# syl051088/DynaAlign

Measured on AMD Instinct MI355X. Metric: sequence-pairs/sec (MinHash k=4 n_hash=500; NW BLOSUM62) at 1/2/4/8 MI355X, higher is better.
Workload: dtype u32

## Files before the change

### dynaalign_amd/csrc/dict_kernels.hip

```cpp
#include "da_common.hpp"
#include <atomic>

namespace da {
namespace {

__global__ __launch_bounds__(256) void k_sig_transpose(const uint32_t *__restrict__ sig, int64_t ld_sig, int64_t n,
                                                       int n_hash, uint32_t *__restrict__ sigT, int64_t ldT) {
  __shared__ uint32_t t[64][65];
  const int64_t i0 = (int64_t)blockIdx.x * 64;
  const int h0 = blockIdx.y * 64;
  const int lx = threadIdx.x & 63, ly = threadIdx.x >> 6;
  for (int r = ly; r < 64; r += 4) {
    const int64_t i = i0 + r;
    const int h = h0 + lx;
    t[r][lx] = (i < n && h < n_hash) ? sig[i * ld_sig + h] : 0u;
  }
  __syncthreads();
  for (int r = ly; r < 64; r += 4) {
    const int h = h0 + r;
    const int64_t i = i0 + lx;
    if (h < n_hash && i < ldT) sigT[(int64_t)h * ldT + i] = t[lx][r];
  }
}

constexpr int DK_THREADS = 1024;
constexpr int DK_SLOTS = 16384;
constexpr int DK_PART_KEYS = 8192;
constexpr int DK_MAX_PARTS = 16;

__device__ __forceinline__ uint32_t dk_mix(uint32_t x) {
  x ^= x >> 16; x *= 0x85ebca6bu; x ^= x >> 13; x *= 0xc2b2ae35u; x ^= x >> 16;
  return x;
}
__device__ __forceinline__ int dk_part(uint32_t z, int R) { return (int)__umulhi(z, (uint32_t)R); }
__device__ __forceinline__ uint32_t dk_slot(uint32_t z) { return (z * 0x9e3779b1u) >> (32 - 14); }
static_assert(DK_SLOTS == (1 << 14), "dk_slot assumes 2^14 slots");

__global__ __launch_bounds__(DK_THREADS) void k_dictionary(const uint32_t *__restrict__ sigT, int64_t ldT, int64_t n,
                                                           int R, uint32_t *__restrict__ szT, uint32_t *__restrict__ siT,
                                                           uint16_t *__restrict__ idsT, int64_t ld_ids,
                                                           int *__restrict__ status) {
  constexpr int NW = DK_THREADS / 64;
  __shared__ uint32_t keys[DK_SLOTS];
  __shared__ uint16_t vals[DK_SLOTS];
  __shared__ uint32_t wsum[NW];
  __shared__ uint32_t cnt[NW][DK_MAX_PARTS];
  __shared__ uint32_t pbase[DK_MAX_PARTS + 1];
  const int tid = threadIdx.x, lane = tid & 63, wave = tid >> 6;
  const uint32_t *col = sigT + (int64_t)blockIdx.x * ldT;
  uint32_t *sz = szT + (int64_t)blockIdx.x * ldT;
  uint32_t *si = siT + (int64_t)blockIdx.x * ldT;
  uint16_t *ids = idsT + (int64_t)blockIdx.x * ld_ids;

  for (int t = tid; t < NW * DK_MAX_PARTS; t += DK_THREADS) (&cnt[0][0])[t] = 0;
  __syncthreads();
  for (int64_t i = tid; i < n; i += DK_THREADS) atomicAdd(&cnt[wave][dk_part(dk_mix(col[i]), R)], 1u);
  __syncthreads();
  if (tid < R) {
    uint32_t run = 0;
    for (int w = 0; w < NW; ++w) { const uint32_t c = cnt[w][tid]; cnt[w][tid] = run; run += c; }
    pbase[tid + 1] = run;
  }
  __syncthreads();
  if (tid == 0) {
    pbase[0] = 0;
    for (int p = 0; p < R; ++p) pbase[p + 1] += pbase[p];
  }
  __syncthreads();
  for (int64_t i = tid; i < n; i += DK_THREADS) {
    const uint32_t z = dk_mix(col[i]);
    const int p = dk_part(z, R);
    const uint32_t pos = pbase[p] + atomicAdd(&cnt[wave][p], 1u);
    sz[pos] = z;
    si[pos] = (uint32_t)i;
  }
  __syncthreads();

  uint32_t base = 0;
  bool overflow = false;
  for (int r = 0; r < R; ++r) {
    const uint32_t lo = pbase[r], hi = pbase[r + 1];
    const uint32_t q = (uint32_t)((r + 1) % R);
    const uint32_t EMPTY = (uint32_t)((((uint64_t)q << 32) + (uint32_t)R - 1) / (uint32_t)R);
    for (int s = tid; s < DK_SLOTS; s += DK_THREADS) { keys[s] = EMPTY; vals[s] = 0; }
    __syncthreads();
    for (uint32_t j = lo + tid; j < hi; j += DK_THREADS) {
      const uint32_t z = sz[j];
      uint32_t s = dk_slot(z);
      for (int probes = 0;; ++probes) {
        const uint32_t old = atomicCAS(&keys[s], EMPTY, z);
        if (old == EMPTY) break;
        if (old == z) { vals[s] = 1; break; }
        s = (s + 1) & (DK_SLOTS - 1);
        if (probes >= DK_SLOTS) { overflow = true; break; }
      }
    }
    __syncthreads();

    uint32_t mine = 0;
    for (int s = tid; s < DK_SLOTS; s += DK_THREADS) mine += vals[s];
    uint32_t incl = mine;
    for (int o = 1; o < 64; o <<= 1) {
      const uint32_t up = __shfl_up(incl, o);
      if (lane >= o) incl += up;
    }
    if (lane == 63) wsum[wave] = incl;
    __syncthreads();
    uint32_t before = 0, total = 0;
    for (int w = 0; w < NW; ++w) {
      const uint32_t v = wsum[w];
      if (w < wave) before += v;
      total += v;
    }
    uint32_t next = base + before + incl - mine;
    for (int s = tid; s < DK_SLOTS; s += DK_THREADS) {
      if (keys[s] == EMPTY) continue;
      vals[s] = vals[s] ? (uint16_t)(next++) : (uint16_t)0xFFFFu;
    }
    base += total;
    __syncthreads();

    for (uint32_t j = lo + tid; j < hi; j += DK_THREADS) {
      const uint32_t z = sz[j];
      uint32_t s = dk_slot(z);
      uint16_t id = 0xFFFFu;
      for (int probes = 0; probes <= DK_SLOTS; ++probes) {
        const uint32_t cur = keys[s];
        if (cur == z) { id = vals[s]; break; }
        if (cur == EMPTY) break;
        s = (s + 1) & (DK_SLOTS - 1);
      }
      ids[si[j]] = id;
    }
    __syncthreads();
  }
  if (overflow) atomicMax(status, 1);
  if (tid == 0 && base > 65534u) atomicMax(status, 2);
  if (tid == 0) atomicMax(status + 1, (int)base);
}

__global__ __launch_bounds__(1024) void k_hy_split(const uint16_t *__restrict__ idsT, int64_t ld_ids, int n, int max_ids, int keep,
                                                   uint16_t *__restrict__ idsD, uint16_t *__restrict__ idsS, unsigned long long *__restrict__ stats) {
  extern __shared__ uint32_t hy_hist[];
  uint32_t *part = hy_hist + max_ids;
  __shared__ uint32_t red[16];
  const int tid = threadIdx.x, lane = tid & 63, wave = tid >> 6;
  const uint16_t *ids = idsT + (int64_t)blockIdx.x * ld_ids;
  uint16_t *outD = idsD + (int64_t)blockIdx.x * ld_ids, *outS = idsS + (int64_t)blockIdx.x * ld_ids;
  for (int c = tid; c < max_ids; c += 1024) hy_hist[c] = 0;
  __syncthreads();
  const uint4 *ids8 = reinterpret_cast<const uint4 *>(ids);
  const int n8 = (n + 7) / 8;
  for (int q = tid; q < n8; q += 1024) {
    const uint4 v = ids8[q];
    const uint32_t w[4] = {v.x, v.y, v.z, v.w};
#pragma unroll
    for (int u = 0; u < 8; ++u) {
      const uint32_t c = (w[u >> 1] >> (16 * (u & 1))) & 0xffffu;
      if (q * 8 + u < n && c != 0xFFFFu) atomicAdd(&hy_hist[c], 1u);
    }
  }
  __syncthreads();
  auto count_ge = [&](uint32_t t) -> uint32_t {
    uint32_t k = 0;
    for (int c = tid; c < max_ids; c += 1024) k += hy_hist[c] >= t;
    for (int o = 32; o > 0; o >>= 1) k += __shfl_down(k, o);
    __syncthreads();
    if (lane == 0) red[wave] = k;
    __syncthreads();
    uint32_t tot = 0;
    for (int w = 0; w < 16; ++w) tot += red[w];
    return tot;
  };
  uint32_t lo = 1, hi = (uint32_t)n + 1u;
  while (lo < hi) {
    const uint32_t mid = lo + (hi - lo) / 2;
    if (count_ge(mid) <= (uint32_t)keep) hi = mid; else lo = mid + 1;
  }
  const uint32_t t = lo, above = count_ge(t), quota = (uint32_t)keep - above;
  const bool ties = t >= 3;
  const int per = (max_ids + 1023) / 1024, c_lo = tid * per, c_hi = c_lo + per < max_ids ? c_lo + per : max_ids;
  uint32_t f1 = 0, f2 = 0;
  for (int c = c_lo; c < c_hi; ++c) { const uint32_t m = hy_hist[c]; f1 += m >= t; f2 += ties && m == t - 1; }
  part[tid] = (f1 << 16) | f2;
  __syncthreads();
  if (tid < 64) {
    uint32_t v[16], tot = 0;
#pragma unroll
    for (int q = 0; q < 16; ++q) { v[q] = part[tid * 16 + q]; tot += v[q]; }
    uint32_t incl = tot;
    for (int o = 1; o < 64; o <<= 1) { const uint32_t up = __shfl_up(incl, o); if (tid >= o) incl += up; }
    uint32_t run = incl - tot;
#pragma unroll
    for (int q = 0; q < 16; ++q) { part[tid * 16 + q] = run; run += v[q]; }
  }
  __syncthreads();
  uint32_t p1 = part[tid] >> 16, p2 = part[tid] & 0xffffu;
  unsigned long long e = 0, mx = 0, e_all = 0, mx_all = 0;
  for (int c = c_lo; c < c_hi; ++c) {
    const uint32_t m = hy_hist[c];
    uint32_t rank = 0xFFFFu;
    if (m >= t) rank = p1++;
    else if (ties && m == t - 1) { if (p2 < quota) rank = above + p2; ++p2; }
    if (m >= 2) {
      const unsigned long long inc = (unsigned long long)m * (m - 1) / 2;
      e_all += inc; mx_all = m > mx_all ? m : mx_all;
      if (rank == 0xFFFFu) { e += inc; mx = m > mx ? m : mx; }
    }
    hy_hist[c] = rank;
  }
  for (int o = 32; o > 0; o >>= 1) {
    e += __shfl_down(e, o);
    e_all += __shfl_down(e_all, o);
    const unsigned long long other = __shfl_down(mx, o), other_all = __shfl_down(mx_all, o);
    mx = other > mx ? other : mx;
    mx_all = other_all > mx_all ? other_all : mx_all;
  }
  if (lane == 0) { atomicAdd(&stats[0], e); atomicMax(&stats[1], mx); atomicAdd(&stats[2], e_all); atomicMax(&stats[3], mx_all); }
  __syncthreads();
  uint4 *outD8 = reinterpret_cast<uint4 *>(outD), *outS8 = reinterpret_cast<uint4 *>(outS);
  for (int q = tid; q < n8; q += 1024) {
    const uint4 v = ids8[q];
    const uint32_t w[4] = {v.x, v.y, v.z, v.w};
    uint32_t d[4] = {0, 0, 0, 0}, sp[4] = {0, 0, 0, 0};
#pragma unroll
    for (int u = 0; u < 8; ++u) {
      const uint32_t c = (w[u >> 1] >> (16 * (u & 1))) & 0xffffu;
      const bool live = q * 8 + u < n && c != 0xFFFFu;
      const uint32_t r = live ? hy_hist[c] : 0xFFFFu;
      d[u >> 1] |= r << (16 * (u & 1));
      sp[u >> 1] |= ((live && r == 0xFFFFu) ? c : 0xFFFFu) << (16 * (u & 1));
    }
    outD8[q] = make_uint4(d[0], d[1], d[2], d[3]);
    outS8[q] = make_uint4(sp[0], sp[1], sp[2], sp[3]);
  }
}

__global__ __launch_bounds__(256) void k_ids_to_planes(const uint16_t *__restrict__ idsT, int64_t ld_ids, int64_t n,
                                                       int n_hash, int pl, int code_bits, uint32_t *__restrict__ planes) {
  __shared__ uint16_t tile[64][66];
  const int64_t i0 = (int64_t)blockIdx.x * 64;
  const int lane = threadIdx.x & 63, wave = threadIdx.x >> 6;
  const PlaneGeom pg = plane_geom(n, n_hash, pl);
  const int ngroup = (n_hash + 31) / 32;
  for (int h0 = 0; h0 < ngroup * 32; h0 += 64) {
    __syncthreads();
    for (int r = wave; r < 64; r += 4) {
      const int h = h0 + r;
      const int64_t i = i0 + lane;
      tile[r][lane] = (h < n_hash && i < n) ? idsT[(int64_t)h * ld_ids + i] : (uint16_t)0;
    }
    __syncthreads();
    for (int sq = wave; sq < 64; sq += 4) {
      const int64_t i = i0 + sq;
      if (i >= n) break;
      const uint32_t v = tile[lane][sq];
      const bool single = (v == 0xFFFFu) && (h0 + lane < n_hash);
      const uint32_t va = single ? (1u << code_bits) - 2u : v;
      const uint32_t vb = single ? (1u << code_bits) - 1u : v;
      uint32_t wa = 0, wb = 0;
      for (int p = 0; p < pl; ++p) {
        const unsigned long long m = __ballot((va >> p) & 1u);
        const uint32_t half = (lane < 32) ? (uint32_t)m : (uint32_t)(m >> 32);
        wa = ((lane & 31) == p) ? half : wa;
      }
      {
        const unsigned long long m = __ballot(vb & 1u);
        const uint32_t half = (lane < 32) ? (uint32_t)m : (uint32_t)(m >> 32);
        wb = ((lane & 31) == 0) ? half : wa;
      }
      const int g = (h0 >> 5) + (lane >> 5);
      const int p = lane & 31;
      if (p < pl && g < ngroup) {
        const int64_t w = plane_unit_word(pg, i, g, p >> 2);
        planes[w + (p & 3)] = wa;
        planes[pg.copy_words + w + ((p & 3) ^ 1)] = wb;
        if (pl == 16) {
          const int64_t ws = pad16_base_words(n, n_hash) + pad16_slot_word(n, n_hash, i, g);
          planes[ws + p] = wa;
          planes[ws + pad16_copy_words(n, n_hash) + (p ^ 1)] = wb;
        }
      }
    }
  }
}

__global__ __launch_bounds__(256) void k_sig_to_planes(const uint32_t *__restrict__ sig, int64_t ld_sig, int64_t n,
                                                       int n_hash, uint32_t *__restrict__ planes) {
  const int lane = threadIdx.x & 63, wave = threadIdx.x >> 6;
  const int64_t i = (int64_t)blockIdx.x * 4 + wave;
  if (i >= n) return;
  const PlaneGeom pg = plane_geom(n, n_hash, 32);
  const int ngroup = (n_hash + 31) / 32;
  const uint32_t *row = sig + i * ld_sig;
  for (int h0 = 0; h0 < ngroup * 32; h0 += 64) {
    const int h = h0 + lane;
    const uint32_t v = (h < n_hash) ? row[h] : 0u;
    uint32_t w = 0;
#pragma unroll
    for (int p = 0; p < 32; ++p) {
      const unsigned long long m = __ballot((v >> p) & 1u);
      const uint32_t half = (lane < 32) ? (uint32_t)m : (uint32_t)(m >> 32);
      w = ((lane & 31) == p) ? half : w;
    }
    const int g = (h0 >> 5) + (lane >> 5);
    const int p = lane & 31;
    if (g < ngroup) {
      const int64_t u = plane_unit_word(pg, i, 2 * g + (p >> 4), (p & 15) >> 2);
      planes[u + (p & 3)] = w;
      planes[pg.copy_words + u + ((p & 3) ^ 1)] = w;
    }
  }
}

}

static int64_t dict_ldT(int64_t n) { return ceil_div(n, 64) * 64; }

struct DictWork { uint32_t *sigT, *sz, *si; uint16_t *idsT; int *status; };
static DictWork dict_work(void *d_work, int64_t n, int n_hash) {
  const size_t m = (size_t)n_hash * (size_t)dict_ldT(n);
  DictWork w;
  w.sigT = static_cast<uint32_t *>(d_work);
  w.sz = w.sigT + m;
  w.si = w.sz + m;
  w.idsT = reinterpret_cast<uint16_t *>(w.si + m);
  w.status = reinterpret_cast<int *>((reinterpret_cast<uintptr_t>(w.idsT + m) + 63) & ~(uintptr_t)63);
  return w;
}

size_t mh_planes_workspace_bytes(int64_t n, int n_hash) {
  if (n <= 0 || n_hash <= 0 || n > DA_DICT_MAX_N) return 256;
  const size_t ldT = (size_t)dict_ldT(n);
  return (size_t)n_hash * ldT * (4 + 4 + 4 + 2) + 256;
}

const uint16_t *mh_dictionary_codes(const void *d_work, int64_t n, int n_hash, int64_t *ld_ids) {
  *ld_ids = dict_ldT(n);
  return dict_work(const_cast<void *>(d_work), n, n_hash).idsT;
}

int launch_mh_dictionary(const uint32_t *d_sig, int64_t ld_sig, int64_t n, int n_hash, void *d_work,
                         int **d_status_out, hipStream_t stream) {
  const int64_t ldT = dict_ldT(n);
  const DictWork w = dict_work(d_work, n, n_hash);
  uint32_t *sigT = w.sigT;
  uint16_t *idsT = w.idsT;
  int *status = w.status;
  *d_status_out = status;
  DA_HIP_TRY(hipMemsetAsync(status, 0, 2 * sizeof(int), stream));
  hipLaunchKernelGGL(k_sig_transpose, dim3((unsigned)ceil_div(n, 64), (unsigned)ceil_div(n_hash, 64)), dim3(256), 0,
                     stream, d_sig, ld_sig, n, n_hash, sigT, ldT);
  int R = (int)ceil_div(n, DK_PART_KEYS);
  if (R < 2) R = 2;
  hipLaunchKernelGGL(k_dictionary, dim3((unsigned)n_hash), dim3(DK_THREADS), 0, stream, sigT, ldT, n, R, w.sz, w.si, idsT, ldT,
                     status);
  DA_HIP_TRY(hipGetLastError());
  return DA_OK;
}

constexpr int HY_MAX_IDS = 32768;
int launch_mh_heavy_split(void *d_work, int64_t n, int n_hash, int max_ids, int keep, const uint16_t **d_dense_out, const uint16_t **d_sparse_out,
                          unsigned long long *d_stats, hipStream_t stream) {
  if (max_ids < 1 || max_ids > HY_MAX_IDS || keep < 1 || keep > 65534 || n > 0x7fffffffLL)
    return fail(DA_ERR_UNSUPPORTED, "heavy / rare split: too many repeated values per column");
  const int64_t ldT = dict_ldT(n);
  const DictWork w = dict_work(d_work, n, n_hash);
  uint16_t *dense = reinterpret_cast<uint16_t *>(w.sz), *sparse = reinterpret_cast<uint16_t *>(w.si);
  static std::atomic<uint64_t> attr_done;
  int dev = 0;
  DA_HIP_TRY(hipGetDevice(&dev));
  if (!((attr_done.load() >> (dev & 63)) & 1u)) {
    DA_HIP_TRY(hipFuncSetAttribute(reinterpret_cast<const void *>(k_hy_split), hipFuncAttributeMaxDynamicSharedMemorySize, (HY_MAX_IDS + 1024) * 4));
    attr_done.fetch_or(1ull << (dev & 63));
  }
  DA_HIP_TRY(hipMemsetAsync(d_stats, 0, 32, stream));
  hipLaunchKernelGGL(k_hy_split, dim3((unsigned)n_hash), dim3(1024), (size_t)(max_ids + 1024) * 4, stream, w.idsT, ldT, (int)n, max_ids, keep, dense, sparse,
                     d_stats);
  DA_HIP_TRY(hipGetLastError());
  *d_dense_out = dense;
  *d_sparse_out = sparse;
  return DA_OK;
}

int mh_plane_bits_for(int max_ids) {
  if (max_ids + 2 <= (1 << 8)) return 8;
  if (max_ids + 2 <= (1 << 12)) return 12;
  if (max_ids + 2 <= (1 << 14)) return 14;
  if (max_ids + 2 <= (1 << 15)) return 15;
  return 16;
}

int launch_ids_to_planes(const void *d_work, int64_t n, int n_hash, int plane_bits, uint32_t *d_planes,
                         hipStream_t stream, const uint16_t *d_codes) {
  const int64_t ldT = dict_ldT(n);
  const uint16_t *idsT = d_codes ? d_codes : dict_work(const_cast<void *>(d_work), n, n_hash).idsT;
  hipLaunchKernelGGL(k_ids_to_planes, dim3((unsigned)ceil_div(n, 64)), dim3(256), 0, stream, idsT, ldT, n, n_hash,
                     (plane_bits == 14 || plane_bits == 15) ? 16 : plane_bits, plane_bits, d_planes);
  DA_HIP_TRY(hipGetLastError());
  return DA_OK;
}

int launch_sig_to_planes(const uint32_t *d_sig, int64_t ld_sig, int64_t n, int n_hash, uint32_t *d_planes,
                         hipStream_t stream) {
  hipLaunchKernelGGL(k_sig_to_planes, dim3((unsigned)ceil_div(n, 4)), dim3(256), 0, stream, d_sig, ld_sig, n, n_hash,
                     d_planes);
  DA_HIP_TRY(hipGetLastError());
  return DA_OK;
}

}
```

Before: 355.3 billion.

## Vectorize and batch global loads in dictionary build and ids-to-planes transpose

Replaces the scalar strided global reads in the dictionary kernel's histogram, scatter, insert and emit phases with batched uint4 loads. Several loads are issued before processing so more memory requests are in flight, and unaligned head and tail elements get separate handling. The ids-to-planes kernel now loads 16-byte units and prefetches the next 64-row tile into registers while the current one is processed. DK_MAX_PARTS is now derived from DA_DICT_MAX_N. Risks include misaligned vector loads if the leading dimensions are not multiples of four, reading past n into padding in the planes kernel, and higher register pressure.

```diff
diff --git a/dynaalign_amd/csrc/dict_kernels.hip b/dynaalign_amd/csrc/dict_kernels.hip
--- a/dynaalign_amd/csrc/dict_kernels.hip
+++ b/dynaalign_amd/csrc/dict_kernels.hip
@@ -24,17 +24,19 @@
 }
 
 constexpr int DK_THREADS = 1024;
-constexpr int DK_SLOTS = 16384;
-constexpr int DK_PART_KEYS = 8192;
-constexpr int DK_MAX_PARTS = 16;
+constexpr int DK_SLOT_BITS = 14;
+constexpr int DK_SLOTS = 1 << DK_SLOT_BITS;
+constexpr int DK_PART_KEYS = DK_SLOTS / 2;
+constexpr int DK_MAX_PARTS = (DA_DICT_MAX_N + DK_PART_KEYS - 1) / DK_PART_KEYS;
+constexpr int DK_COL_BATCH = 8;
+constexpr int DK_PART_BATCH = 4;
 
 __device__ __forceinline__ uint32_t dk_mix(uint32_t x) {
   x ^= x >> 16; x *= 0x85ebca6bu; x ^= x >> 13; x *= 0xc2b2ae35u; x ^= x >> 16;
   return x;
 }
 __device__ __forceinline__ int dk_part(uint32_t z, int R) { return (int)__umulhi(z, (uint32_t)R); }
-__device__ __forceinline__ uint32_t dk_slot(uint32_t z) { return (z * 0x9e3779b1u) >> (32 - 14); }
-static_assert(DK_SLOTS == (1 << 14), "dk_slot assumes 2^14 slots");
+__device__ __forceinline__ uint32_t dk_slot(uint32_t z) { return (z * 0x9e3779b1u) >> (32 - DK_SLOT_BITS); }
 
 __global__ __launch_bounds__(DK_THREADS) void k_dictionary(const uint32_t *__restrict__ sigT, int64_t ldT, int64_t n,
                                                            int R, uint32_t *__restrict__ szT, uint32_t *__restrict__ siT,
@@ -54,7 +56,25 @@
 
   for (int t = tid; t < NW * DK_MAX_PARTS; t += DK_THREADS) (&cnt[0][0])[t] = 0;
   __syncthreads();
-  for (int64_t i = tid; i < n; i += DK_THREADS) atomicAdd(&cnt[wave][dk_part(dk_mix(col[i]), R)], 1u);
+  const uint4 *col4 = reinterpret_cast<const uint4 *>(col);
+  const int nv = (int)(n >> 2);
+  const int n_tail = (int)n - 4 * nv;
+  for (int q0 = 0; q0 < nv; q0 += DK_THREADS * DK_COL_BATCH) {
+    uint4 v[DK_COL_BATCH];
+#pragma unroll
+    for (int b = 0; b < DK_COL_BATCH; ++b) {
+      const int q = q0 + b * DK_THREADS + tid;
+      v[b] = col4[q < nv ? q : 0];
+    }
+#pragma unroll
+    for (int b = 0; b < DK_COL_BATCH; ++b) {
+      if (q0 + b * DK_THREADS + tid >= nv) continue;
+      const uint32_t x[4] = {v[b].x, v[b].y, v[b].z, v[b].w};
+#pragma unroll
+      for (int c = 0; c < 4; ++c) atomicAdd(&cnt[wave][dk_part(dk_mix(x[c]), R)], 1u);
+    }
+  }
+  if (tid < n_tail) atomicAdd(&cnt[wave][dk_part(dk_mix(col[4 * nv + tid]), R)], 1u);
   __syncthreads();
   if (tid < R) {
     uint32_t run = 0;
@@ -67,13 +87,30 @@
     for (int p = 0; p < R; ++p) pbase[p + 1] += pbase[p];
   }
   __syncthreads();
-  for (int64_t i = tid; i < n; i += DK_THREADS) {
-    const uint32_t z = dk_mix(col[i]);
+  auto scatter = [&](uint32_t x, uint32_t i) {
+    const uint32_t z = dk_mix(x);
     const int p = dk_part(z, R);
     const uint32_t pos = pbase[p] + atomicAdd(&cnt[wave][p], 1u);
     sz[pos] = z;
-    si[pos] = (uint32_t)i;
-  }
+    si[pos] = i;
+  };
+  for (int q0 = 0; q0 < nv; q0 += DK_THREADS * DK_COL_BATCH) {
+    uint4 v[DK_COL_BATCH];
+#pragma unroll
+    for (int b = 0; b < DK_COL_BATCH; ++b) {
+      const int q = q0 + b * DK_THREADS + tid;
+      v[b] = col4[q < nv ? q : 0];
+    }
+#pragma unroll
+    for (int b = 0; b < DK_COL_BATCH; ++b) {
+      const int q = q0 + b * DK_THREADS + tid;
+      if (q >= nv) continue;
+      const uint32_t x[4] = {v[b].x, v[b].y, v[b].z, v[b].w};
+#pragma unroll
+      for (int c = 0; c < 4; ++c) scatter(x[c], (uint32_t)(4 * q + c));
+    }
+  }
+  if (tid < n_tail) scatter(col[4 * nv + tid], (uint32_t)(4 * nv + tid));
   __syncthreads();
 
   uint32_t base = 0;
@@ -84,9 +121,15 @@
     const uint32_t EMPTY = (uint32_t)((((uint64_t)q << 32) + (uint32_t)R - 1) / (uint32_t)R);
     for (int s = tid; s < DK_SLOTS; s += DK_THREADS) { keys[s] = EMPTY; vals[s] = 0; }
     __syncthreads();
-    for (uint32_t j = lo + tid; j < hi; j += DK_THREADS) {
-      const uint32_t z = sz[j];
+    const uint32_t va = ((lo + 3u) & ~3u) < hi ? ((lo + 3u) & ~3u) : hi;
+    const uint32_t vb = va + ((hi - va) & ~3u);
+    const int pv0 = (int)(va >> 2), pnv = (int)((vb - va) >> 2);
+    const uint32_t n_head = va - lo, n_ends = n_head + (hi - vb);
+    const uint32_t j_end = (uint32_t)tid < n_head ? lo + tid : vb + (tid - n_head);
+    const uint4 *sz4 = reinterpret_cast<const uint4 *>(sz), *si4 = reinterpret_cast<const uint4 *>(si);
+    auto insert = [&](uint32_t z) {
       uint32_t s = dk_slot(z);
+#pragma unroll 1
       for (int probes = 0;; ++probes) {
         const uint32_t old = atomicCAS(&keys[s], EMPTY, z);
         if (old == EMPTY) break;
@@ -94,7 +137,21 @@
         s = (s + 1) & (DK_SLOTS - 1);
         if (probes >= DK_SLOTS) { overflow = true; break; }
       }
-    }
+    };
+    for (int q0 = 0; q0 < pnv; q0 += DK_THREADS * DK_PART_BATCH) {
+      uint4 v[DK_PART_BATCH];
+#pragma unroll
+      for (int b = 0; b < DK_PART_BATCH; ++b) {
+        const int q = q0 + b * DK_THREADS + tid;
+        v[b] = sz4[pv0 + (q < pnv ? q : 0)];
+      }
+#pragma unroll
+      for (int b = 0; b < DK_PART_BATCH; ++b) {
+        if (q0 + b * DK_THREADS + tid >= pnv) continue;
+        insert(v[b].x); insert(v[b].y); insert(v[b].z); insert(v[b].w);
+      }
+    }
+    if ((uint32_t)tid < n_ends) insert(sz[j_end]);
     __syncthreads();
 
     uint32_t mine = 0;
@@ -120,17 +177,35 @@
     base += total;
     __syncthreads();
 
-    for (uint32_t j = lo + tid; j < hi; j += DK_THREADS) {
-      const uint32_t z = sz[j];
+    auto emit = [&](uint32_t z, uint32_t i) {
       uint32_t s = dk_slot(z);
       uint16_t id = 0xFFFFu;
+#pragma unroll 1
       for (int probes = 0; probes <= DK_SLOTS; ++probes) {
         const uint32_t cur = keys[s];
         if (cur == z) { id = vals[s]; break; }
         if (cur == EMPTY) break;
         s = (s + 1) & (DK_SLOTS - 1);
       }
-      ids[si[j]] = id;
+      ids[i] = id;
+    };
+    for (int q0 = 0; q0 < pnv; q0 += DK_THREADS * DK_PART_BATCH) {
+      uint4 v[DK_PART_BATCH], w[DK_PART_BATCH];
+#pragma unroll
+      for (int b = 0; b < DK_PART_BATCH; ++b) {
+        const int q = q0 + b * DK_THREADS + tid;
+        v[b] = sz4[pv0 + (q < pnv ? q : 0)];
+        w[b] = si4[pv0 + (q < pnv ? q : 0)];
+      }
+#pragma unroll
+      for (int b = 0; b < DK_PART_BATCH; ++b) {
+        if (q0 + b * DK_THREADS + tid >= pnv) continue;
+        emit(v[b].x, w[b].x); emit(v[b].y, w[b].y); emit(v[b].z, w[b].z); emit(v[b].w, w[b].w);
+      }
+    }
+    if ((uint32_t)tid < n_ends) {
+      const uint32_t z = sz[j_end], i = si[j_end];
+      emit(z, i);
     }
     __syncthreads();
   }
@@ -243,13 +318,24 @@
   const int lane = threadIdx.x & 63, wave = threadIdx.x >> 6;
   const PlaneGeom pg = plane_geom(n, n_hash, pl);
   const int ngroup = (n_hash + 31) / 32;
+  auto load_units = [&](int h0, uint4 (&u)[2]) {
+#pragma unroll
+    for (int k = 0; k < 2; ++k) {
+      const int unit = (int)threadIdx.x + 256 * k, h = h0 + (unit >> 3);
+      u[k] = h < n_hash ? *reinterpret_cast<const uint4 *>(idsT + (int64_t)h * ld_ids + i0 + 8 * (unit & 7)) : make_uint4(0, 0, 0, 0);
+    }
+  };
+  uint4 nx[2];
+  load_units(0, nx);
   for (int h0 = 0; h0 < ngroup * 32; h0 += 64) {
     __syncthreads();
-    for (int r = wave; r < 64; r += 4) {
-      const int h = h0 + r;
-      const int64_t i = i0 + lane;
-      tile[r][lane] = (h < n_hash && i < n) ? idsT[(int64_t)h * ld_ids + i] : (uint16_t)0;
-    }
+#pragma unroll
+    for (int k = 0; k < 2; ++k) {
+      const int unit = (int)threadIdx.x + 256 * k;
+      uint32_t *dst = reinterpret_cast<uint32_t *>(&tile[unit >> 3][8 * (unit & 7)]);
+      dst[0] = nx[k].x; dst[1] = nx[k].y; dst[2] = nx[k].z; dst[3] = nx[k].w;
+    }
+    if (h0 + 64 < ngroup * 32) load_units(h0 + 64, nx);
     __syncthreads();
     for (int sq = wave; sq < 64; sq += 4) {
       const int64_t i = i0 + sq;
```

Result: no change. 356.4 billion (median of 2 runs) (+0.3%).
